# JuliaSmoothOptimizers/LinearOperators.jl

Hardware: AMD Instinct MI355X
Metric: mul! GB/s (frac HBM peak) at n=10^8 fp64; L-BFGS apply/s, 1/2/4/8 GPU (higher is better)
Workload: dtype f64; 1 GPU; opHouseholder(h) 5-arg mul!(res,H,v,1,0), n=100000000 fp64 per GPU (configs[1]); n_per_gpu=100000000, algorithmic_bytes_per_elt=40, devices_visible=1

## Files before the change

### linearoperators.jl_amd/csrc/common.h

```cpp
#pragma once
#include <hip/hip_runtime.h>
#include <atomic>

#include <cstdarg>
#include <cstdint>
#include <cstdio>
#include <cstdlib>
#include <cstring>
#include <initializer_list>
#include <type_traits>
#include <utility>
#include <vector>

#include "../../include/mxlo.h"

#define MXLO_API extern "C" __attribute__((visibility("default")))

namespace mxlo {

constexpr int kBlock = 256;
constexpr int kWave = 64;
constexpr int kMaxRedCols = 128;
constexpr int kQnfMaxCols = 40, kQnfMaxGrid = 256;
constexpr int kQnfSlots = kQnfMaxCols * kQnfMaxGrid;
constexpr int kFusedSlots = 512;
constexpr unsigned long long kSlotEmpty = 0x7FF8DEADBEEF0001ull;
constexpr int kMaxRedBlocks = 4096;
constexpr int kScalarSlots = 8192;

void set_error(const char *fmt, ...);

struct ApiCounters {
  std::atomic<int64_t> n_malloc{0}, n_free{0}, n_h2d{0}, n_d2h{0}, n_d2d{0}, n_d2h_bytes{0}, n_stream_sync{0},
      n_device_sync{0}, n_event_sync{0}, n_memset_async{0}, n_launch{0}, n_blocking_copy{0};
};
inline ApiCounters &api_counters() {
  static ApiCounters c;
  return c;
}
inline void count_copy(size_t bytes, hipMemcpyKind kind, bool blocking) {
  ApiCounters &c = api_counters();
  if (kind == hipMemcpyDeviceToHost) { ++c.n_d2h; c.n_d2h_bytes += (int64_t)bytes; }
  else if (kind == hipMemcpyHostToDevice) ++c.n_h2d;
  else ++c.n_d2d;
  if (blocking) ++c.n_blocking_copy;
}
inline hipError_t counted_memcpy(void *d, const void *s, size_t b, hipMemcpyKind k) {
  count_copy(b, k, true);
  return hipMemcpy(d, s, b, k);
}
inline hipError_t counted_memcpy_async(void *d, const void *s, size_t b, hipMemcpyKind k, hipStream_t st) {
  count_copy(b, k, false);
  return hipMemcpyAsync(d, s, b, k, st);
}
#define hipMalloc(...) (++mxlo::api_counters().n_malloc, hipMalloc(__VA_ARGS__))
#define hipFree(...) (++mxlo::api_counters().n_free, hipFree(__VA_ARGS__))
#define hipHostMalloc(...) (++mxlo::api_counters().n_malloc, hipHostMalloc(__VA_ARGS__))
#define hipHostFree(...) (++mxlo::api_counters().n_free, hipHostFree(__VA_ARGS__))
#define hipMemcpy(...) mxlo::counted_memcpy(__VA_ARGS__)
#define hipMemcpyAsync(...) mxlo::counted_memcpy_async(__VA_ARGS__)
#define hipStreamSynchronize(...) (++mxlo::api_counters().n_stream_sync, hipStreamSynchronize(__VA_ARGS__))
#define hipDeviceSynchronize(...) (++mxlo::api_counters().n_device_sync, hipDeviceSynchronize(__VA_ARGS__))
#define hipEventSynchronize(...) (++mxlo::api_counters().n_event_sync, hipEventSynchronize(__VA_ARGS__))
#define hipMemsetAsync(...) (++mxlo::api_counters().n_memset_async, hipMemsetAsync(__VA_ARGS__))

#define MXLO_HIP(call)                                                                           \
  do {                                                                                           \
    hipError_t e__ = (call);                                                                     \
    if (e__ != hipSuccess) {                                                                     \
      mxlo::set_error("%s failed: %s (%s:%d)", #call, hipGetErrorString(e__), __FILE__, __LINE__); \
      return MXLO_EHIP;                                                                          \
    }                                                                                            \
  } while (0)

#define MXLO_REQUIRE(cond, code, ...)                                                            \
  do {                                                                                           \
    if (!(cond)) {                                                                               \
      mxlo::set_error(__VA_ARGS__);                                                              \
      return (code);                                                                             \
    }                                                                                            \
  } while (0)

#define MXLO_TRY(expr)                                                                           \
  do {                                                                                           \
    int32_t s__ = (expr);                                                                        \
    if (s__ != MXLO_OK) return s__;                                                              \
  } while (0)

inline bool mxlo_trace_on() {
  static const bool on = getenv("MXLO_TRACE") != nullptr;
  return on;
}
#define MXLO_LAUNCH_CHECK()                                                                      \
  do {                                                                                           \
    ++mxlo::api_counters().n_launch;                                                             \
    if (mxlo_trace_on()) {                                                                       \
      fprintf(stderr, "[mxlo] launched %s:%d ... ", __FILE__, __LINE__);                         \
      fflush(stderr);                                                                            \
      (void)hipDeviceSynchronize();                                                              \
      fprintf(stderr, "done\n");                                                                 \
    }                                                                                            \
    hipError_t e__ = hipGetLastError();                                                          \
    if (e__ != hipSuccess) {                                                                     \
      mxlo::set_error("kernel launch failed: %s (%s:%d)", hipGetErrorString(e__), __FILE__,      \
                      __LINE__);                                                                 \
      return MXLO_EHIP;                                                                          \
    }                                                                                            \
  } while (0)
// ... 287 lines not shown
```

### linearoperators.jl_amd/csrc/house_keep.h

```cpp
#pragma once
#include "common.h"
#include "house_keep_plan.h"
#include "stream_kernels.h"

namespace mxlo {

constexpr int kHouseKeepKR = 14;
constexpr int kHouseKeepKL = 4;
constexpr int kHouseKeepUnroll = 4;

template <typename T, typename CA, typename CB, bool BETA0, int KR, int KL>
__global__ void __launch_bounds__(kBlock)
householder_dots_keep_kernel(T *__restrict__ res, const T *__restrict__ h, const T *__restrict__ v, int64_t head,
                             int64_t n, CA alpha, CB beta, HouseKeepPlan pl, unsigned long long *__restrict__ slots,
                             unsigned long long ticks, unsigned *__restrict__ fault, int drop,
                             double *__restrict__ dot_out) {
  constexpr int VEC = Vec16<T>::N, U = kHouseKeepUnroll;
  using V = typename Vec16<T>::type;
  constexpr int64_t CHUNK = (int64_t)kBlock * U;
  extern __shared__ __attribute__((aligned(16))) unsigned char keep_lds[];
  V *lh = reinterpret_cast<V *>(keep_lds), *lx = lh + (int64_t)KL * CHUNK;
  const int tid = threadIdx.x, G = (int)gridDim.x, b = (int)blockIdx.x;
  unsigned long long *epoch = slots + 2 * kFusedSlots;
  const unsigned e = (unsigned)__hip_atomic_load(epoch, __ATOMIC_RELAXED, __HIP_MEMORY_SCOPE_AGENT) & 1u;
  unsigned long long *mine = slots + e * kFusedSlots, *other = slots + (1u - e) * kFusedSlots;
  for (int i = b + tid * G; i < kFusedSlots; i += G * kBlock)
    __hip_atomic_store(other + i, kSlotEmpty, __ATOMIC_RELAXED, __HIP_MEMORY_SCOPE_AGENT);

  const V *hv = reinterpret_cast<const V *>(h + head), *xv = reinterpret_cast<const V *>(v + head);
  V *rv = reinterpret_cast<V *>(res + head);
  double acc = 0.0;
  auto load4 = [&](int64_t round, V (&a)[U], V (&x)[U]) {
    const int64_t base = (round * G + b) * CHUNK + tid;
#pragma unroll
    for (int u = 0; u < U; ++u) {
      x[u] = __builtin_nontemporal_load(xv + base + (int64_t)u * kBlock);
      a[u] = __builtin_nontemporal_load(hv + base + (int64_t)u * kBlock);
    }
  };
  auto fma4 = [&](const V (&a)[U], const V (&x)[U]) {
#pragma unroll
    for (int u = 0; u < U; ++u)
#pragma unroll
      for (int k = 0; k < VEC; ++k) acc = fma((double)a[u][k], (double)x[u][k], acc);
  };
  for (int64_t r = 0; r < pl.first; ++r) {
    V a[U], x[U];
    load4(r, a, x);
    fma4(a, x);
  }
  if constexpr (KL > 0) {
#pragma unroll 1
    for (int q = 0; q < pl.kl; ++q) {
      V a[U], x[U];
      load4(pl.first + q, a, x);
      fma4(a, x);
#pragma unroll
      for (int u = 0; u < U; ++u) {
        lh[(q * U + u) * kBlock + tid] = a[u];
        lx[(q * U + u) * kBlock + tid] = x[u];
      }
    }
  }
  V kh[KR][U], kx[KR][U];
  const int64_t reg0 = pl.first + pl.kl;
#pragma unroll
  for (int q = 0; q < KR; ++q)
    if (q < pl.kr) load4(reg0 + q, kh[q], kx[q]);
#pragma unroll
  for (int q = 0; q < KR; ++q)
    if (q < pl.kr) fma4(kh[q], kx[q]);
  const int64_t rem = pl.rem_vec + (int64_t)b * CHUNK + tid;
#pragma unroll
  for (int u = 0; u < U; ++u) {
    const int64_t i = rem + (int64_t)u * kBlock;
    if (i < pl.nvec) {
      const V x = __builtin_nontemporal_load(xv + i), a = __builtin_nontemporal_load(hv + i);
#pragma unroll
      for (int k = 0; k < VEC; ++k) acc = fma((double)a[k], (double)x[k], acc);
    }
  }
  const int64_t tail0 = head + pl.nvec * VEC, cnt = head + (n - tail0);
  if (b == G - 1 && tid < cnt) {
    const int64_t i = tid < head ? tid : tail0 + (tid - head);
    acc = fma((double)h[i], (double)v[i], acc);
  }

  __shared__ double lds[kBlock / kWave];
  const int wave = tid >> 6, lane = tid & 63;
  acc = wave_sum(acc);
  if (lane == 0) lds[wave] = acc;
  __syncthreads();
  if (tid == 0) {
    const double s = (lds[0] + lds[1]) + (lds[2] + lds[3]);
    unsigned long long bits = (unsigned long long)__double_as_longlong(s);
    if (s != s) bits = kCanonicalNaN;
    if (b != drop) __hip_atomic_store(mine + b, bits, __ATOMIC_RELAXED, __HIP_MEMORY_SCOPE_AGENT);
  }
  double p = 0.0;
  for (int i = tid; i < G; i += kBlock) p += __longlong_as_double((long long)poll_slot(mine + i, ticks, fault, kFaultHouseholder));
  p = wave_sum(p);
  __syncthreads();
  if (lane == 0) lds[wave] = p;
  __syncthreads();
  const double dot = (lds[0] + lds[1]) + (lds[2] + lds[3]);
  if (b == 0 && tid == 0) {
    *dot_out = dot;
    __hip_atomic_store(epoch, (unsigned long long)(1u - e), __ATOMIC_RELAXED, __HIP_MEMORY_SCOPE_AGENT);
  }

  HouseholderOp<T, CA, CB, BETA0> op{alpha, beta, nullptr, T(0)};
  op.c = (T)2 * (T)dot;
  auto update4 = [&](int64_t round, const V (&a)[U], const V (&x)[U]) {
    const int64_t base = (round * G + b) * CHUNK + tid;
    V r[U];
    if constexpr (!BETA0) {
#pragma unroll
      for (int u = 0; u < U; ++u) r[u] = __builtin_nontemporal_load(rv + base + (int64_t)u * kBlock);
    }
#pragma unroll
    for (int u = 0; u < U; ++u) {
      V o;
#pragma unroll
      for (int k = 0; k < VEC; ++k) o[k] = op(a[u][k], x[u][k], BETA0 ? T(0) : r[u][k]);
      __builtin_nontemporal_store(o, rv + base + (int64_t)u * kBlock);
    }
  };
#pragma unroll
  for (int q = 0; q < KR; ++q)
    if (q < pl.kr) update4(reg0 + q, kh[q], kx[q]);
  if constexpr (KL > 0) {
#pragma unroll 1
    for (int q = 0; q < pl.kl; ++q) {
      V a[U], x[U];
#pragma unroll
      for (int u = 0; u < U; ++u) {
        a[u] = lh[(q * U + u) * kBlock + tid];
        x[u] = lx[(q * U + u) * kBlock + tid];
      }
      update4(pl.first + q, a, x);
    }
  }
#pragma unroll
  for (int u = 0; u < U; ++u) {
    const int64_t i = rem + (int64_t)u * kBlock;
    if (i < pl.nvec) {
      const V x = xv[i], a = hv[i];
      V r, o;
      if constexpr (!BETA0) r = rv[i];
#pragma unroll
      for (int k = 0; k < VEC; ++k) o[k] = op(a[k], x[k], BETA0 ? T(0) : r[k]);
      __builtin_nontemporal_store(o, rv + i);
    }
  }
  if (b == G - 1 && tid >= head && tid < cnt) {
    const int64_t i = tail0 + (tid - head);
    res[i] = op(h[i], v[i], BETA0 ? T(0) : res[i]);
  }
}

template <typename T>
static int32_t householder_dots_t(mxlo_ctx *ctx, T *res, const T *h, const T *v, int64_t *n_left, double alpha,
                                  double beta, int32_t flags, double *dot) {
  constexpr int VEC = Vec16<T>::N, KR = kHouseKeepKR, KL = kHouseKeepKL;
  constexpr int64_t CHUNK = (int64_t)kBlock * kHouseKeepUnroll;
  constexpr size_t kLds = (size_t)2 * KL * CHUNK * 16;
  const int64_t n = *n_left;
  const T *cols[1] = {h};
  const int64_t head = common_head<T>({res, h, v});
  bool keep = ctx->tune.house_fused && !ctx->allreduce && ctx->fault_dev && n > ctx->tune.house_inline_n && head >= 0 &&
              n >= 4 * VEC && (int64_t)sizeof(T) * n * 2 >= ctx->tune.nt_min_bytes;
  HouseKeepPlan pl;
  int grid = 0;
  if (keep) {
    const int per_cu = ctx->tune.red_blocks_per_cu > 1 ? 1 : ctx->tune.red_blocks_per_cu;
    grid = grid_for(ctx, (n - head) / VEC, CHUNK, per_cu);
    pl = house_keep_plan(n, head, VEC, grid, CHUNK, KR, KL);
    keep = grid == ctx->num_cu && grid <= kFusedSlots && pl.ok;
  }
  if (!keep) return panel_dots<T>(ctx, cols, 1, v, n, dot);
  bool launched = false;
  MXLO_TRY((dispatch_ab<T>(beta, flags, [&]<typename CA, typename CB, bool B0>() -> int32_t {
    constexpr auto kernel = householder_dots_keep_kernel<T, CA, CB, B0, KR, KL>;
    static std::atomic<int> lds_cap[64];
    const int d = ctx->device & 63;
    int st = kLds > 48 * 1024 ? lds_cap[d].load(std::memory_order_relaxed) : 1;
    if (st == 0) {
      st = hipFuncSetAttribute((const void *)kernel, hipFuncAttributeMaxDynamicSharedMemorySize, (int)kLds) == hipSuccess ? 1 : 2;
      if (st == 2) (void)hipGetLastError();
      lds_cap[d].store(st, std::memory_order_relaxed);
    }
    if (st != 1 || !coresident<kernel>(ctx, grid, kLds)) return MXLO_OK;
    hipLaunchKernelGGL(kernel, dim3(grid), dim3(kBlock), kLds, ctx->stream, res, h, v, head, n, (CA)alpha, (CB)beta, pl,
                       ctx->xslots, fused_timeout_ticks(ctx), ctx->fault_dev, ctx->tune.fused_debug_drop, dot);
    MXLO_LAUNCH_CHECK();
    launched = true;
    return MXLO_OK;
  })));
  if (!launched) return panel_dots<T>(ctx, cols, 1, v, n, dot);
  *n_left = pl.prefix;
  return MXLO_OK;
}

}
```

### linearoperators.jl_amd/csrc/house_keep_plan.h

```cpp
#pragma once
#include <cstdint>

namespace mxlo {

struct HouseKeepPlan {
  bool ok = false;
  int64_t rounds = 0;
  int64_t first = 0;
  int kl = 0, kr = 0;
  int64_t prefix = 0;
  int64_t rem_vec = 0;
  int64_t nvec = 0;
};

inline HouseKeepPlan house_keep_plan(int64_t n, int64_t head, int vec, int64_t grid, int64_t chunk, int KR, int KL) {
  HouseKeepPlan p;
  if (n < head || vec < 1 || grid < 1 || chunk < 1 || KR < 0 || KL < 0) return p;
  p.nvec = (n - head) / vec;
  p.rounds = p.nvec / chunk / grid;
  if (p.rounds < 2) return p;
  const int64_t kept = p.rounds - 1 < (int64_t)KR + KL ? p.rounds - 1 : (int64_t)KR + KL;
  p.kr = (int)(kept < KR ? kept : KR);
  p.kl = (int)(kept - p.kr);
  p.first = p.rounds - kept;
  p.prefix = head + p.first * grid * chunk * vec;
  p.rem_vec = p.rounds * grid * chunk;
  p.ok = kept >= 1;
  return p;
}

}
```

### linearoperators.jl_amd/csrc/leaves.hip

```cpp
#include "common.h"
#include "stream_kernels.h"
#include "house_keep.h"
using namespace mxlo;

#define CHECK_COMMON(name)                                                                       \
  MXLO_REQUIRE(ctx != nullptr, MXLO_EINVAL, name ": ctx is NULL");                               \
  MXLO_REQUIRE(dtype == MXLO_F64 || dtype == MXLO_F32, MXLO_EINVAL, name ": bad dtype %d", dtype)

static inline double eff_beta(int32_t dtype, int32_t flags, double beta) {
  return beta_is_f64(dtype == MXLO_F64 ? 8 : 4, flags) ? beta : (double)(float)beta;
}
static inline double eff_alpha(int32_t dtype, int32_t flags, double alpha) {
  return alpha_is_f64(dtype == MXLO_F64 ? 8 : 4, flags) ? alpha : (double)(float)alpha;
}

template <typename T>
static int32_t fill(mxlo_ctx *ctx, T *p, int64_t n, T c) {
  if (n <= 0) return MXLO_OK;
  if (c == T(0)) {
    MXLO_HIP(hipMemsetAsync(p, 0, sizeof(T) * (size_t)n, ctx->stream));
    return MXLO_OK;
  }
  return launch_map<T, 0, false, false>(ctx, p, (const T *)nullptr, (const T *)nullptr, n,
                                        FillOp<T>{c});
// ... 113 lines not shown
}

namespace {
template <typename T>
__global__ void __launch_bounds__(kBlock)
sum_kernel(const T *__restrict__ v, int64_t n, double *__restrict__ partials) {
  constexpr int VEC = Vec16<T>::N;
  using V = typename Vec16<T>::type;
  double acc = 0.0;
  const int64_t head = (((uintptr_t)v & 15u) == 0) ? 0 : n;
  const int64_t nvec = head == 0 ? n / VEC : 0;
  const V *vv = reinterpret_cast<const V *>(v);
  const int64_t stride = (int64_t)gridDim.x * kBlock;
  int64_t i = (int64_t)blockIdx.x * kBlock + threadIdx.x;
  for (; i + 3 * stride < nvec; i += 4 * stride) {
    const V a = __builtin_nontemporal_load(vv + i), b = __builtin_nontemporal_load(vv + i + stride),
            c = __builtin_nontemporal_load(vv + i + 2 * stride), d = __builtin_nontemporal_load(vv + i + 3 * stride);
#pragma unroll
    for (int e = 0; e < VEC; ++e) acc += ((double)a[e] + (double)b[e]) + ((double)c[e] + (double)d[e]);
  }
  for (; i < nvec; i += stride) {
    const V a = vv[i];
#pragma unroll
    for (int e = 0; e < VEC; ++e) acc += (double)a[e];
  }
  for (int64_t k = nvec * VEC + (int64_t)blockIdx.x * kBlock + threadIdx.x; k < n; k += stride) acc += (double)v[k];
#pragma unroll
  for (int off = 32; off > 0; off >>= 1) acc += __shfl_down(acc, off, 64);
  __shared__ double lds[kBlock / kWave];
  if ((threadIdx.x & 63) == 0) lds[threadIdx.x >> 6] = acc;
  __syncthreads();
  if (threadIdx.x == 0) partials[blockIdx.x] = (lds[0] + lds[1]) + (lds[2] + lds[3]);
}
}

namespace mxlo {
int32_t allreduce_hook(mxlo_ctx *ctx, double *dev, int64_t count);
}

template <typename T>
static int32_t ones_mul_t(mxlo_ctx *ctx, T *res, int64_t nrow, const T *v, int64_t ncol,
                          double alpha, double beta, int32_t flags) {
  double *sum = ctx->scalars;
  if (ncol > 0) {
    const int grid = grid_for(ctx, ncol, kBlock * 8, ctx->tune.red_blocks_per_cu);
    hipLaunchKernelGGL((sum_kernel<T>), dim3(grid), dim3(kBlock), 0, ctx->stream, v, ncol,
                       ctx->partials);
    MXLO_LAUNCH_CHECK();
    MXLO_TRY(finalize_and_reduce(ctx, 1, grid, sum));
  } else {
    MXLO_HIP(hipMemsetAsync(sum, 0, sizeof(double), ctx->stream));
  }
  MXLO_TRY(allreduce_hook(ctx, sum, 1));
  return dispatch_ab<T>(beta, flags, [&]<typename CA, typename CB, bool B0>() -> int32_t {
    OnesOp<T, CA, CB, B0> op{(CA)alpha, (CB)beta, sum, (CA)0};
    return launch_map<T, 0, !B0, false>(ctx, res, (const T *)nullptr, (const T *)nullptr, nrow, op);
  });
}

MXLO_API int32_t mxlo_ones_mul(mxlo_ctx *ctx, int32_t dtype, void *res, int64_t nrow,
                               const void *v, int64_t ncol, double alpha, double beta,
                               int32_t flags) {
  CHECK_COMMON("mxlo_ones_mul");
  MXLO_DEVICE_GUARD(ctx);
  MXLO_REQUIRE(nrow >= 0 && ncol >= 0, MXLO_ESHAPE, "mxlo_ones_mul: negative size");
  alpha = eff_alpha(dtype, flags, alpha);
  beta = eff_beta(dtype, flags, beta);
  if (dtype == MXLO_F64)
    return ones_mul_t<double>(ctx, (double *)res, nrow, (const double *)v, ncol, alpha, beta, flags);
  return ones_mul_t<float>(ctx, (float *)res, nrow, (const float *)v, ncol, alpha, beta, flags);
}

template <typename T>
static int32_t householder_apply_t(mxlo_ctx *ctx, T *res, const T *h, const T *v, int64_t n,
                                   double alpha, double beta, int32_t flags, const double *dot) {
  const bool rev = ctx->tune.house_reverse != 0;
  return dispatch_ab<T>(beta, flags, [&]<typename CA, typename CB, bool B0>() -> int32_t {
    HouseholderOp<T, CA, CB, B0> op{(CA)alpha, (CB)beta, dot, T(0)};
    if (rev) return launch_map<T, 2, !B0, true>(ctx, res, h, v, n, op);
    return launch_map<T, 2, !B0, false>(ctx, res, h, v, n, op);
  });
}

namespace {
template <typename T, typename CA, typename CB, bool BETA0, int VPT, bool ALIGNED>
__global__ void __launch_bounds__(kBlock)
householder_fused_kernel(T *__restrict__ res, const T *__restrict__ h, const T *__restrict__ v, int64_t n, CA alpha,
                         CB beta, unsigned long long *__restrict__ slots, unsigned long long ticks,
                         unsigned *__restrict__ fault, int drop) {
  constexpr int VEC = Vec16<T>::N;
  using V = typename Vec16<T>::type;
  const int tid = threadIdx.x, G = (int)gridDim.x, b = (int)blockIdx.x;
  unsigned long long *epoch = slots + 2 * kFusedSlots;
  const unsigned e = (unsigned)__hip_atomic_load(epoch, __ATOMIC_RELAXED, __HIP_MEMORY_SCOPE_AGENT) & 1u;
  unsigned long long *mine = slots + e * kFusedSlots, *other = slots + (1u - e) * kFusedSlots;
  for (int i = b + tid * G; i < kFusedSlots; i += G * kBlock)
    __hip_atomic_store(other + i, kSlotEmpty, __ATOMIC_RELAXED, __HIP_MEMORY_SCOPE_AGENT);

  T hh[VPT][VEC], vv[VPT][VEC];
  double acc = 0.0;
  const int64_t base = (int64_t)b * kBlock * VPT * VEC;
#pragma unroll
  for (int q = 0; q < VPT; ++q) {
    const int64_t i = base + ((int64_t)q * kBlock + tid) * VEC;
    if (ALIGNED && i + VEC <= n) {
      const V a = *reinterpret_cast<const V *>(h + i), c = *reinterpret_cast<const V *>(v + i);
#pragma unroll
      for (int k = 0; k < VEC; ++k) { hh[q][k] = a[k]; vv[q][k] = c[k]; }
    } else {
#pragma unroll
      for (int k = 0; k < VEC; ++k) {
        hh[q][k] = i + k < n ? h[i + k] : T(0);
        vv[q][k] = i + k < n ? v[i + k] : T(0);
      }
    }
  }
#pragma unroll
  for (int q = 0; q < VPT; ++q)
#pragma unroll
    for (int k = 0; k < VEC; ++k) acc = fma((double)hh[q][k], (double)vv[q][k], acc);

  __shared__ double lds[kBlock / 64];
  const int wave = tid >> 6, lane = tid & 63;
#pragma unroll
  for (int off = 32; off > 0; off >>= 1) acc += __shfl_down(acc, off, 64);
  if (lane == 0) lds[wave] = acc;
  __syncthreads();
  if (tid == 0) {
    const double s = (lds[0] + lds[1]) + (lds[2] + lds[3]);
    unsigned long long bits = (unsigned long long)__double_as_longlong(s);
    if (s != s) bits = kCanonicalNaN;
    if (b != drop) __hip_atomic_store(mine + b, bits, __ATOMIC_RELAXED, __HIP_MEMORY_SCOPE_AGENT);
  }
  double p = 0.0;
  if (tid < G) p = __longlong_as_double((long long)poll_slot(mine + tid, ticks, fault, kFaultHouseholder));
  if (tid + kBlock < G) p += __longlong_as_double((long long)poll_slot(mine + tid + kBlock, ticks, fault, kFaultHouseholder));
#pragma unroll
  for (int off = 32; off > 0; off >>= 1) p += __shfl_down(p, off, 64);
  __syncthreads();
  if (lane == 0) lds[wave] = p;
  __syncthreads();
  const double dot = (lds[0] + lds[1]) + (lds[2] + lds[3]);
  if (b == 0 && tid == 0)
    __hip_atomic_store(epoch, (unsigned long long)(1u - e), __ATOMIC_RELAXED, __HIP_MEMORY_SCOPE_AGENT);

  HouseholderOp<T, CA, CB, BETA0> op{alpha, beta, nullptr, T(0)};
  op.c = (T)2 * (T)dot;
#pragma unroll
  for (int q = 0; q < VPT; ++q) {
    const int64_t i = base + ((int64_t)q * kBlock + tid) * VEC;
    if (ALIGNED && i + VEC <= n) {
      V r;
      if constexpr (!BETA0) r = *reinterpret_cast<const V *>(res + i);
      V o;
#pragma unroll
      for (int k = 0; k < VEC; ++k) o[k] = op(hh[q][k], vv[q][k], BETA0 ? T(0) : r[k]);
      *reinterpret_cast<V *>(res + i) = o;
    } else {
#pragma unroll
      for (int k = 0; k < VEC; ++k)
        if (i + k < n) res[i + k] = op(hh[q][k], vv[q][k], BETA0 ? T(0) : res[i + k]);
    }
  }
}
}

template <typename T>
static inline int64_t fused_grid(int64_t n, int vpt) {
  const int64_t per = (int64_t)kBlock * vpt * Vec16<T>::N;
  return (n + per - 1) / per;
}

template <typename T>
static int32_t householder_fused_t(mxlo_ctx *ctx, T *res, const T *h, const T *v, int64_t n, double alpha, double beta,
                                   int32_t flags, int vpt, bool *launched) {
  const bool aligned = ((((uintptr_t)res) | ((uintptr_t)h) | ((uintptr_t)v)) & 15u) == 0;
  const int grid = (int)fused_grid<T>(n, vpt);
  return dispatch_ab<T>(beta, flags, [&]<typename CA, typename CB, bool B0>() -> int32_t {
    bool fits = true;
    auto go = [&]<int VPT, bool AL>() {
      if (!(fits = coresident<householder_fused_kernel<T, CA, CB, B0, VPT, AL>>(ctx, grid))) return;
      hipLaunchKernelGGL((householder_fused_kernel<T, CA, CB, B0, VPT, AL>), dim3(grid), dim3(kBlock), 0, ctx->stream,
                         res, h, v, n, (CA)alpha, (CB)beta, ctx->xslots, fused_timeout_ticks(ctx), ctx->fault_dev,
                         ctx->tune.fused_debug_drop);
    };
    if (aligned) {
      if (vpt == 2) go.template operator()<2, true>();
      else if (vpt == 4) go.template operator()<4, true>();
      else if (vpt == 8) go.template operator()<8, true>();
      else go.template operator()<16, true>();
    } else {
      if (vpt == 2) go.template operator()<2, false>();
      else if (vpt == 4) go.template operator()<4, false>();
      else if (vpt == 8) go.template operator()<8, false>();
      else go.template operator()<16, false>();
    }
    *launched = fits;
    if (!fits) return MXLO_OK;
    MXLO_LAUNCH_CHECK();
    return MXLO_OK;
  });
}

template <typename T>
static int32_t householder_t(mxlo_ctx *ctx, T *res, const T *h, const T *v, int64_t n,
                             double alpha, double beta, int32_t flags) {
  if (ctx->tune.house_fused && !ctx->allreduce && n > 0 && ctx->fault_dev) {
    MXLO_TRY(fused_fault_check(ctx));
  }
  if (ctx->tune.house_fused && !ctx->allreduce && n > 0 && ctx->fault_dev) {
    const int64_t cap = std::min<int64_t>((int64_t)ctx->num_cu * (ctx->tune.house_fused_per_cu >= 2 ? 2 : 1), kFusedSlots);
    const int64_t cap1 = std::min<int64_t>(ctx->num_cu, kFusedSlots);
    const int vpt = fused_grid<T>(n, 2) <= 16 ? 2 : (fused_grid<T>(n, 4) <= 32 ? 4 : (fused_grid<T>(n, 8) <= cap1 ? 8 : 16));
    if (fused_grid<T>(n, vpt) <= cap) {
      bool launched = false;
      const int32_t st = householder_fused_t<T>(ctx, res, h, v, n, alpha, beta, flags, vpt, &launched);
      if (st != MXLO_OK || launched) return st;
    }
  }
  const T *cols[1] = {h};
  if (!ctx->allreduce && n >= 1 && n <= ctx->tune.house_inline_n) {
    int nb = 0;
    MXLO_TRY(panel_dots_partials<T>(ctx, cols, 1, v, n, &nb));
    const bool rev = ctx->tune.house_reverse != 0;
    return dispatch_ab<T>(beta, flags, [&]<typename CA, typename CB, bool B0>() -> int32_t {
      HouseholderPartialsOp<T, CA, CB, B0> op{(CA)alpha, (CB)beta, ctx->partials, nb, T(0)};
      if (rev) return launch_map<T, 2, !B0, true>(ctx, res, h, v, n, op);
      return launch_map<T, 2, !B0, false>(ctx, res, h, v, n, op);
    });
  }
  double *dot = ctx->scalars;
  MXLO_TRY(householder_dots_t<T>(ctx, res, h, v, &n, alpha, beta, flags, dot));
  return householder_apply_t<T>(ctx, res, h, v, n, alpha, beta, flags, dot);
}

MXLO_API int32_t mxlo_dot(mxlo_ctx *ctx, int32_t dtype, const void *a, const void *b, int64_t n,
                          double *out_dev) {
  CHECK_COMMON("mxlo_dot");
  MXLO_DEVICE_GUARD(ctx);
  MXLO_REQUIRE(n >= 0 && out_dev && (n == 0 || (a && b)), MXLO_EINVAL, "mxlo_dot: bad argument");
  if (dtype == MXLO_F64) {
    const double *cols[1] = {(const double *)a};
    return panel_dots<double>(ctx, cols, 1, (const double *)b, n, out_dev);
  }
  const float *cols[1] = {(const float *)a};
  return panel_dots<float>(ctx, cols, 1, (const float *)b, n, out_dev);
}

MXLO_API int32_t mxlo_householder_apply(mxlo_ctx *ctx, int32_t dtype, void *res, const void *h,
                                        const void *v, int64_t n, double alpha, double beta,
                                        int32_t flags, const double *dot_dev) {
  CHECK_COMMON("mxlo_householder_apply");
  MXLO_DEVICE_GUARD(ctx);
  MXLO_REQUIRE(n >= 0 && dot_dev && (n == 0 || (res && h && v)), MXLO_EINVAL,
               "mxlo_householder_apply: bad argument");
  MXLO_TRY(stage_alias(ctx, res, n * (dtype == MXLO_F64 ? 8 : 4), &v, n * (dtype == MXLO_F64 ? 8 : 4), true,
                       "mxlo_householder_apply"));
  alpha = eff_alpha(dtype, flags, alpha);
  beta = eff_beta(dtype, flags, beta);
  if (dtype == MXLO_F64)
    return householder_apply_t<double>(ctx, (double *)res, (const double *)h, (const double *)v, n,
                                       alpha, beta, flags, dot_dev);
  return householder_apply_t<float>(ctx, (float *)res, (const float *)h, (const float *)v, n, alpha,
                                    beta, flags, dot_dev);
}

MXLO_API int32_t mxlo_householder_mul(mxlo_ctx *ctx, int32_t dtype, void *res, const void *h,
                                      const void *v, int64_t n, double alpha, double beta,
                                      int32_t flags) {
  CHECK_COMMON("mxlo_householder_mul");
  MXLO_DEVICE_GUARD(ctx);
  MXLO_REQUIRE(n >= 0 && (n == 0 || (res && h && v)), MXLO_EINVAL,
               "mxlo_householder_mul: bad argument");
  MXLO_TRY(stage_alias(ctx, res, n * (dtype == MXLO_F64 ? 8 : 4), &v, n * (dtype == MXLO_F64 ? 8 : 4), true,
                       "mxlo_householder_mul"));
  alpha = eff_alpha(dtype, flags, alpha);
  beta = eff_beta(dtype, flags, beta);
  if (dtype == MXLO_F64)
    return householder_t<double>(ctx, (double *)res, (const double *)h, (const double *)v, n, alpha,
                                 beta, flags);
  return householder_t<float>(ctx, (float *)res, (const float *)h, (const float *)v, n, alpha, beta,
                              flags);
}

namespace {
template <typename T>
struct CopyBitsOp {
  __device__ void init() {}
  __device__ T operator()(T x, T, T) const { return x; }
};

typedef unsigned int u32;
typedef unsigned long long u64;
typedef u64 u64x2 __attribute__((ext_vector_type(2)));

template <typename E, bool VECOUT>
__global__ void __launch_bounds__(kBlock)
gather_idx_kernel(E *__restrict__ res, const E *__restrict__ v, const int64_t *__restrict__ idx,
                  int64_t nidx) {
  constexpr int KPT = sizeof(E) >= 16 ? 1 : 16 / (int)sizeof(E);
  constexpr int U = 4;
  typedef long long i64x2 __attribute__((ext_vector_type(2)));
  const int64_t ngroups = (nidx + KPT - 1) / KPT;
  const bool idx_al = (((uintptr_t)idx) & 15u) == 0;
  for (int64_t base = ((int64_t)blockIdx.x * U) * kBlock + threadIdx.x; base < ngroups;
       base += (int64_t)gridDim.x * U * kBlock) {
    int64_t j[U][KPT];
#pragma unroll
    for (int u = 0; u < U; ++u) {
      const int64_t k0 = (base + (int64_t)u * kBlock) * KPT;
      if (KPT >= 2 && idx_al && k0 + KPT <= nidx) {
#pragma unroll
        for (int q = 0; q < KPT; q += 2) {
          const i64x2 t = __builtin_nontemporal_load(reinterpret_cast<const i64x2 *>(idx + k0 + q));
          j[u][q] = t[0] - 1;
          j[u][q + (KPT >= 2 ? 1 : 0)] = t[1] - 1;
// ... 631 lines not shown
```

Baseline: 6989 GB/s.

## Extend keep-in-register Householder kernel to non-temporal-free sizes with virtual-grid accumulators

Generalises the single-pass Householder kernel so a grid pinned to one workgroup per CU can emulate a larger virtual grid. Each block keeps 2 or 4 partial accumulators, selected per round through branchless blends, and publishes one exchange slot per virtual block. Non-temporal loads and stores become a template option, so mid-size inputs below the non-temporal threshold can also use the fused dot-plus-update path instead of a separate dot and apply. The slot array is doubled and the fused-grid cap is decoupled from it. Large inputs keep the previous single-accumulator non-temporal configuration.

```diff
diff --git a/linearoperators.jl_amd/csrc/common.h b/linearoperators.jl_amd/csrc/common.h
--- a/linearoperators.jl_amd/csrc/common.h
+++ b/linearoperators.jl_amd/csrc/common.h
@@ -23,7 +23,7 @@
 constexpr int kMaxRedCols = 128;
 constexpr int kQnfMaxCols = 40, kQnfMaxGrid = 256;
 constexpr int kQnfSlots = kQnfMaxCols * kQnfMaxGrid;
-constexpr int kFusedSlots = 512;
+constexpr int kFusedSlots = 1024;
 constexpr unsigned long long kSlotEmpty = 0x7FF8DEADBEEF0001ull;
 constexpr int kMaxRedBlocks = 4096;
 constexpr int kScalarSlots = 8192;
diff --git a/linearoperators.jl_amd/csrc/house_keep.h b/linearoperators.jl_amd/csrc/house_keep.h
--- a/linearoperators.jl_amd/csrc/house_keep.h
+++ b/linearoperators.jl_amd/csrc/house_keep.h
@@ -9,12 +9,13 @@
 constexpr int kHouseKeepKL = 4;
 constexpr int kHouseKeepUnroll = 4;
 
-template <typename T, typename CA, typename CB, bool BETA0, int KR, int KL>
+template <typename T, typename CA, typename CB, bool BETA0, int KR, int KL, int NV, bool NT>
 __global__ void __launch_bounds__(kBlock)
 householder_dots_keep_kernel(T *__restrict__ res, const T *__restrict__ h, const T *__restrict__ v, int64_t head,
                              int64_t n, CA alpha, CB beta, HouseKeepPlan pl, unsigned long long *__restrict__ slots,
                              unsigned long long ticks, unsigned *__restrict__ fault, int drop,
                              double *__restrict__ dot_out) {
+  static_assert(NV == 1 || NV == 2 || NV == 4, "accumulators per workgroup");
   constexpr int VEC = Vec16<T>::N, U = kHouseKeepUnroll;
   using V = typename Vec16<T>::type;
   constexpr int64_t CHUNK = (int64_t)kBlock * U;
@@ -29,32 +30,91 @@
 
   const V *hv = reinterpret_cast<const V *>(h + head), *xv = reinterpret_cast<const V *>(v + head);
   V *rv = reinterpret_cast<V *>(res + head);
-  double acc = 0.0;
+  auto ld = [](const V *p) -> V {
+    if constexpr (NT) return __builtin_nontemporal_load(p);
+    else return *p;
+  };
+  auto st = [](V o, V *p) {
+    if constexpr (NT) __builtin_nontemporal_store(o, p);
+    else *p = o;
+  };
+  double a0 = 0.0, a1 = 0.0, a2 = 0.0, a3 = 0.0;
+  auto mask = [](int j, int jj) -> unsigned long long {
+    unsigned long long m = j == jj ? ~0ull : 0ull;
+    asm volatile("" : "+v"(m));
+    return m;
+  };
+  auto blend = [](double x, double y, unsigned long long m) -> double {
+    const unsigned long long xb = (unsigned long long)__double_as_longlong(x), yb = (unsigned long long)__double_as_longlong(y);
+    return __longlong_as_double((long long)((yb & m) | (xb & ~m)));
+  };
+  auto pick = [&](int j) -> double {
+    double s = a0;
+    if constexpr (NV >= 2) s = blend(s, a1, mask(j, 1));
+    if constexpr (NV >= 4) {
+      s = blend(s, a2, mask(j, 2));
+      s = blend(s, a3, mask(j, 3));
+    }
+    return s;
+  };
+  auto put = [&](int j, double s) {
+    if constexpr (NV == 1) {
+      a0 = s;
+    } else {
+      a0 = blend(a0, s, mask(j, 0));
+      a1 = blend(a1, s, mask(j, 1));
+      if constexpr (NV >= 4) {
+        a2 = blend(a2, s, mask(j, 2));
+        a3 = blend(a3, s, mask(j, 3));
+      }
+    }
+  };
   auto load4 = [&](int64_t round, V (&a)[U], V (&x)[U]) {
     const int64_t base = (round * G + b) * CHUNK + tid;
 #pragma unroll
     for (int u = 0; u < U; ++u) {
-      x[u] = __builtin_nontemporal_load(xv + base + (int64_t)u * kBlock);
-      a[u] = __builtin_nontemporal_load(hv + base + (int64_t)u * kBlock);
-    }
-  };
-  auto fma4 = [&](const V (&a)[U], const V (&x)[U]) {
+      x[u] = ld(xv + base + (int64_t)u * kBlock);
+      a[u] = ld(hv + base + (int64_t)u * kBlock);
+    }
+  };
+  auto fma4 = [&](const V (&a)[U], const V (&x)[U], double s) -> double {
 #pragma unroll
     for (int u = 0; u < U; ++u)
 #pragma unroll
-      for (int k = 0; k < VEC; ++k) acc = fma((double)a[u][k], (double)x[u][k], acc);
-  };
-  for (int64_t r = 0; r < pl.first; ++r) {
+      for (int k = 0; k < VEC; ++k) s = fma((double)a[u][k], (double)x[u][k], s);
+    return s;
+  };
+  auto fma4_at = [&](int64_t round, const V (&a)[U], const V (&x)[U]) {
+    const int j = house_keep_acc(round, NV);
+    put(j, fma4(a, x, pick(j)));
+  };
+  auto stream = [&](int64_t round, double &s) {
     V a[U], x[U];
-    load4(r, a, x);
-    fma4(a, x);
+    load4(round, a, x);
+    s = fma4(a, x, s);
+  };
+  int64_t r = 0;
+  for (; r + NV <= pl.first; r += NV) {
+    stream(r, a0);
+    if constexpr (NV >= 2) stream(r + 1, a1);
+    if constexpr (NV >= 4) {
+      stream(r + 2, a2);
+      stream(r + 3, a3);
+    }
+  }
+  if constexpr (NV >= 2) {
+    if (r < pl.first) stream(r, a0);
+  }
+  if constexpr (NV >= 4) {
+    if (r + 1 < pl.first) stream(r + 1, a1);
+    if (r + 2 < pl.first) stream(r + 2, a2);
   }
   if constexpr (KL > 0) {
 #pragma unroll 1
     for (int q = 0; q < pl.kl; ++q) {
       V a[U], x[U];
       load4(pl.first + q, a, x);
-      fma4(a, x);
+      fma4_at(pl.first + q, a, x);
 #pragma unroll
       for (int u = 0; u < U; ++u) {
         lh[(q * U + u) * kBlock + tid] = a[u];
@@ -69,41 +129,55 @@
     if (q < pl.kr) load4(reg0 + q, kh[q], kx[q]);
 #pragma unroll
   for (int q = 0; q < KR; ++q)
-    if (q < pl.kr) fma4(kh[q], kx[q]);
+    if (q < pl.kr) fma4_at(reg0 + q, kh[q], kx[q]);
   const int64_t rem = pl.rem_vec + (int64_t)b * CHUNK + tid;
-#pragma unroll
-  for (int u = 0; u < U; ++u) {
-    const int64_t i = rem + (int64_t)u * kBlock;
-    if (i < pl.nvec) {
-      const V x = __builtin_nontemporal_load(xv + i), a = __builtin_nontemporal_load(hv + i);
-#pragma unroll
-      for (int k = 0; k < VEC; ++k) acc = fma((double)a[k], (double)x[k], acc);
-    }
+  {
+    const int jr = house_keep_acc(pl.rounds, NV);
+    double s = pick(jr);
+#pragma unroll
+    for (int u = 0; u < U; ++u) {
+      const int64_t i = rem + (int64_t)u * kBlock;
+      if (i < pl.nvec) {
+        const V x = ld(xv + i), a = ld(hv + i);
+#pragma unroll
+        for (int k = 0; k < VEC; ++k) s = fma((double)a[k], (double)x[k], s);
+      }
+    }
+    put(jr, s);
   }
   const int64_t tail0 = head + pl.nvec * VEC, cnt = head + (n - tail0);
   if (b == G - 1 && tid < cnt) {
     const int64_t i = tid < head ? tid : tail0 + (tid - head);
-    acc = fma((double)h[i], (double)v[i], acc);
-  }
-
-  __shared__ double lds[kBlock / kWave];
+    double &last = NV == 1 ? a0 : (NV == 2 ? a1 : a3);
+    last = fma((double)h[i], (double)v[i], last);
+  }
+
+  __shared__ double lds[NV][kBlock / kWave];
   const int wave = tid >> 6, lane = tid & 63;
-  acc = wave_sum(acc);
-  if (lane == 0) lds[wave] = acc;
+  auto wave_partial = [&](int j, double a) {
+    const double s = wave_sum(a);
+    if (lane == 0) lds[j][wave] = s;
+  };
+  wave_partial(0, a0);
+  if constexpr (NV >= 2) wave_partial(1, a1);
+  if constexpr (NV >= 4) {
+    wave_partial(2, a2);
+    wave_partial(3, a3);
+  }
   __syncthreads();
-  if (tid == 0) {
-    const double s = (lds[0] + lds[1]) + (lds[2] + lds[3]);
+  if (tid < NV) {
+    const double s = (lds[tid][0] + lds[tid][1]) + (lds[tid][2] + lds[tid][3]);
     unsigned long long bits = (unsigned long long)__double_as_longlong(s);
     if (s != s) bits = kCanonicalNaN;
-    if (b != drop) __hip_atomic_store(mine + b, bits, __ATOMIC_RELAXED, __HIP_MEMORY_SCOPE_AGENT);
+    if (b != drop) __hip_atomic_store(mine + house_keep_slot(b, tid, G), bits, __ATOMIC_RELAXED, __HIP_MEMORY_SCOPE_AGENT);
   }
   double p = 0.0;
-  for (int i = tid; i < G; i += kBlock) p += __longlong_as_double((long long)poll_slot(mine + i, ticks, fault, kFaultHouseholder));
+  for (int i = tid; i < NV * G; i += kBlock) p += __longlong_as_double((long long)poll_slot(mine + i, ticks, fault, kFaultHouseholder));
   p = wave_sum(p);
   __syncthreads();
-  if (lane == 0) lds[wave] = p;
+  if (lane == 0) lds[0][wave] = p;
   __syncthreads();
-  const double dot = (lds[0] + lds[1]) + (lds[2] + lds[3]);
+  const double dot = (lds[0][0] + lds[0][1]) + (lds[0][2] + lds[0][3]);
   if (b == 0 && tid == 0) {
     *dot_out = dot;
     __hip_atomic_store(epoch, (unsigned long long)(1u - e), __ATOMIC_RELAXED, __HIP_MEMORY_SCOPE_AGENT);
@@ -113,17 +187,17 @@
   op.c = (T)2 * (T)dot;
   auto update4 = [&](int64_t round, const V (&a)[U], const V (&x)[U]) {
     const int64_t base = (round * G + b) * CHUNK + tid;
-    V r[U];
+    V rr[U];
     if constexpr (!BETA0) {
 #pragma unroll
-      for (int u = 0; u < U; ++u) r[u] = __builtin_nontemporal_load(rv + base + (int64_t)u * kBlock);
+      for (int u = 0; u < U; ++u) rr[u] = ld(rv + base + (int64_t)u * kBlock);
     }
 #pragma unroll
     for (int u = 0; u < U; ++u) {
       V o;
 #pragma unroll
-      for (int k = 0; k < VEC; ++k) o[k] = op(a[u][k], x[u][k], BETA0 ? T(0) : r[u][k]);
-      __builtin_nontemporal_store(o, rv + base + (int64_t)u * kBlock);
+      for (int k = 0; k < VEC; ++k) o[k] = op(a[u][k], x[u][k], BETA0 ? T(0) : rr[u][k]);
+      st(o, rv + base + (int64_t)u * kBlock);
     }
   };
 #pragma unroll
@@ -146,11 +220,11 @@
     const int64_t i = rem + (int64_t)u * kBlock;
     if (i < pl.nvec) {
       const V x = xv[i], a = hv[i];
-      V r, o;
-      if constexpr (!BETA0) r = rv[i];
-#pragma unroll
-      for (int k = 0; k < VEC; ++k) o[k] = op(a[k], x[k], BETA0 ? T(0) : r[k]);
-      __builtin_nontemporal_store(o, rv + i);
+      V rr, o;
+      if constexpr (!BETA0) rr = rv[i];
+#pragma unroll
+      for (int k = 0; k < VEC; ++k) o[k] = op(a[k], x[k], BETA0 ? T(0) : rr[k]);
+      st(o, rv + i);
     }
   }
   if (b == G - 1 && tid >= head && tid < cnt) {
@@ -160,44 +234,49 @@
 }
 
 template <typename T>
-static int32_t householder_dots_t(mxlo_ctx *ctx, T *res, const T *h, const T *v, int64_t *n_left, double alpha,
-                                  double beta, int32_t flags, double *dot) {
+static int32_t householder_keep_t(mxlo_ctx *ctx, T *res, const T *h, const T *v, int64_t *n_left, double alpha,
+                                  double beta, int32_t flags, double *dot, bool above_single, bool *kept) {
   constexpr int VEC = Vec16<T>::N, KR = kHouseKeepKR, KL = kHouseKeepKL;
   constexpr int64_t CHUNK = (int64_t)kBlock * kHouseKeepUnroll;
   constexpr size_t kLds = (size_t)2 * KL * CHUNK * 16;
   const int64_t n = *n_left;
-  const T *cols[1] = {h};
+  *kept = false;
   const int64_t head = common_head<T>({res, h, v});
-  bool keep = ctx->tune.house_fused && !ctx->allreduce && ctx->fault_dev && n > ctx->tune.house_inline_n && head >= 0 &&
-              n >= 4 * VEC && (int64_t)sizeof(T) * n * 2 >= ctx->tune.nt_min_bytes;
-  HouseKeepPlan pl;
-  int grid = 0;
-  if (keep) {
-    const int per_cu = ctx->tune.red_blocks_per_cu > 1 ? 1 : ctx->tune.red_blocks_per_cu;
-    grid = grid_for(ctx, (n - head) / VEC, CHUNK, per_cu);
-    pl = house_keep_plan(n, head, VEC, grid, CHUNK, KR, KL);
-    keep = grid == ctx->num_cu && grid <= kFusedSlots && pl.ok;
-  }
-  if (!keep) return panel_dots<T>(ctx, cols, 1, v, n, dot);
+  if (!(ctx->tune.house_fused && !ctx->allreduce && ctx->fault_dev && head >= 0 && n >= 4 * VEC)) return MXLO_OK;
+  const bool nt = (int64_t)sizeof(T) * n * 2 >= ctx->tune.nt_min_bytes;
+  if (nt ? n <= ctx->tune.house_inline_n : !above_single) return MXLO_OK;
+  const int per_cu = (nt && ctx->tune.red_blocks_per_cu > 1) ? 1 : ctx->tune.red_blocks_per_cu;
+  const int64_t g_virtual = grid_for(ctx, (n - head) / VEC, CHUNK, per_cu);
+  const int grid = ctx->num_cu;
+  const int nv = house_keep_virtual(g_virtual, grid, kFusedSlots);
+  const HouseKeepPlan pl = house_keep_plan(n, head, VEC, grid, CHUNK, KR, KL);
+  if (nv == 0 || (nt && nv != 1) || !pl.ok) return MXLO_OK;
   bool launched = false;
   MXLO_TRY((dispatch_ab<T>(beta, flags, [&]<typename CA, typename CB, bool B0>() -> int32_t {
-    constexpr auto kernel = householder_dots_keep_kernel<T, CA, CB, B0, KR, KL>;
-    static std::atomic<int> lds_cap[64];
-    const int d = ctx->device & 63;
-    int st = kLds > 48 * 1024 ? lds_cap[d].load(std::memory_order_relaxed) : 1;
-    if (st == 0) {
-      st = hipFuncSetAttribute((const void *)kernel, hipFuncAttributeMaxDynamicSharedMemorySize, (int)kLds) == hipSuccess ? 1 : 2;
-      if (st == 2) (void)hipGetLastError();
-      lds_cap[d].store(st, std::memory_order_relaxed);
-    }
-    if (st != 1 || !coresident<kernel>(ctx, grid, kLds)) return MXLO_OK;
-    hipLaunchKernelGGL(kernel, dim3(grid), dim3(kBlock), kLds, ctx->stream, res, h, v, head, n, (CA)alpha, (CB)beta, pl,
-                       ctx->xslots, fused_timeout_ticks(ctx), ctx->fault_dev, ctx->tune.fused_debug_drop, dot);
-    MXLO_LAUNCH_CHECK();
-    launched = true;
-    return MXLO_OK;
+    auto go = [&]<int NV, bool NT>() -> int32_t {
+      constexpr auto kernel = householder_dots_keep_kernel<T, CA, CB, B0, KR, KL, NV, NT>;
+      static std::atomic<int> lds_cap[64];
+      const int d = ctx->device & 63;
+      int st = kLds > 48 * 1024 ? lds_cap[d].load(std::memory_order_relaxed) : 1;
+      if (st == 0) {
+        st = hipFuncSetAttribute((const void *)kernel, hipFuncAttributeMaxDynamicSharedMemorySize, (int)kLds) == hipSuccess ? 1 : 2;
+        if (st == 2) (void)hipGetLastError();
+        lds_cap[d].store(st, std::memory_order_relaxed);
+      }
+      if (st != 1 || !coresident<kernel>(ctx, grid, kLds)) return MXLO_OK;
+      hipLaunchKernelGGL(kernel, dim3(grid), dim3(kBlock), kLds, ctx->stream, res, h, v, head, n, (CA)alpha, (CB)beta, pl,
+                         ctx->xslots, fused_timeout_ticks(ctx), ctx->fault_dev, ctx->tune.fused_debug_drop, dot);
+      MXLO_LAUNCH_CHECK();
+      launched = true;
+      return MXLO_OK;
+    };
+    if (nt) return go.template operator()<1, true>();
+    if (nv == 1) return go.template operator()<1, false>();
+    if (nv == 2) return go.template operator()<2, false>();
+    return go.template operator()<4, false>();
   })));
-  if (!launched) return panel_dots<T>(ctx, cols, 1, v, n, dot);
+  if (!launched) return MXLO_OK;
+  *kept = true;
   *n_left = pl.prefix;
   return MXLO_OK;
 }
diff --git a/linearoperators.jl_amd/csrc/house_keep_plan.h b/linearoperators.jl_amd/csrc/house_keep_plan.h
--- a/linearoperators.jl_amd/csrc/house_keep_plan.h
+++ b/linearoperators.jl_amd/csrc/house_keep_plan.h
@@ -29,4 +29,15 @@
   return p;
 }
 
+
+constexpr int house_keep_virtual(int64_t g_virtual, int64_t grid, int64_t slots) {
+  if (grid < 1 || g_virtual < grid || g_virtual > slots || g_virtual % grid) return 0;
+  const int64_t v = g_virtual / grid;
+  return v == 1 || v == 2 || v == 4 ? (int)v : 0;
 }
+
+constexpr int house_keep_acc(int64_t round, int nv) { return (int)(round & (int64_t)(nv - 1)); }
+
+constexpr int64_t house_keep_slot(int64_t b, int j, int64_t grid) { return b + (int64_t)j * grid; }
+
+}
diff --git a/linearoperators.jl_amd/csrc/leaves.hip b/linearoperators.jl_amd/csrc/leaves.hip
--- a/linearoperators.jl_amd/csrc/leaves.hip
+++ b/linearoperators.jl_amd/csrc/leaves.hip
@@ -219,6 +219,8 @@
   });
 }
 
+constexpr int kFusedMaxGrid = 2 * kBlock;
+static_assert(kFusedMaxGrid <= kFusedSlots, "one exchange slot per workgroup");
 namespace {
 template <typename T, typename CA, typename CB, bool BETA0, int VPT, bool ALIGNED>
 __global__ void __launch_bounds__(kBlock)
@@ -345,16 +347,24 @@
   if (ctx->tune.house_fused && !ctx->allreduce && n > 0 && ctx->fault_dev) {
     MXLO_TRY(fused_fault_check(ctx));
   }
+  bool above_single = false;
   if (ctx->tune.house_fused && !ctx->allreduce && n > 0 && ctx->fault_dev) {
-    const int64_t cap = std::min<int64_t>((int64_t)ctx->num_cu * (ctx->tune.house_fused_per_cu >= 2 ? 2 : 1), kFusedSlots);
-    const int64_t cap1 = std::min<int64_t>(ctx->num_cu, kFusedSlots);
+    const int64_t cap = std::min<int64_t>((int64_t)ctx->num_cu * (ctx->tune.house_fused_per_cu >= 2 ? 2 : 1), kFusedMaxGrid);
+    const int64_t cap1 = std::min<int64_t>(ctx->num_cu, kFusedMaxGrid);
     const int vpt = fused_grid<T>(n, 2) <= 16 ? 2 : (fused_grid<T>(n, 4) <= 32 ? 4 : (fused_grid<T>(n, 8) <= cap1 ? 8 : 16));
     if (fused_grid<T>(n, vpt) <= cap) {
       bool launched = false;
       const int32_t st = householder_fused_t<T>(ctx, res, h, v, n, alpha, beta, flags, vpt, &launched);
       if (st != MXLO_OK || launched) return st;
-    }
-  }
+    } else {
+      above_single = true;
+    }
+  }
+  double *dot = ctx->scalars;
+  bool kept = false;
+  int64_t n_left = n;
+  MXLO_TRY(householder_keep_t<T>(ctx, res, h, v, &n_left, alpha, beta, flags, dot, above_single, &kept));
+  if (kept) return householder_apply_t<T>(ctx, res, h, v, n_left, alpha, beta, flags, dot);
   const T *cols[1] = {h};
   if (!ctx->allreduce && n >= 1 && n <= ctx->tune.house_inline_n) {
     int nb = 0;
@@ -366,8 +376,7 @@
       return launch_map<T, 2, !B0, false>(ctx, res, h, v, n, op);
     });
   }
-  double *dot = ctx->scalars;
-  MXLO_TRY(householder_dots_t<T>(ctx, res, h, v, &n, alpha, beta, flags, dot));
+  MXLO_TRY(panel_dots<T>(ctx, cols, 1, v, n, dot));
   return householder_apply_t<T>(ctx, res, h, v, n, alpha, beta, flags, dot);
 }
 
```

Result: no change. 6986 GB/s (-0.0%).

## Keep a cache-sized fraction of h resident between dot and update passes

Applied to the files above, without the earlier changes.

In the kept-form dot kernel, a diagonal subset of chunks (fraction q/16, sized to the cache budget derived from nt_min_bytes) loads h with normal cached loads instead of nontemporal ones, so those lines can stay in the last-level cache. A new update kernel uses the same chunk-to-diagonal mapping to reread those h chunks through the cache and streams the rest. The aim is to cut HBM reads of h in the second pass. The cost is a branch per chunk, an added dependence on cache retention between launches, and a new update path with a stricter chunk-alignment requirement.

```diff
diff --git a/linearoperators.jl_amd/csrc/house_keep.h b/linearoperators.jl_amd/csrc/house_keep.h
--- a/linearoperators.jl_amd/csrc/house_keep.h
+++ b/linearoperators.jl_amd/csrc/house_keep.h
@@ -8,13 +8,22 @@
 constexpr int kHouseKeepKR = 14;
 constexpr int kHouseKeepKL = 4;
 constexpr int kHouseKeepUnroll = 4;
+static_assert(kHouseKeepUnroll == kStreamUnroll, "the dot launch and the update launch count the same chunks");
+
+constexpr int kHouseResidentNum = 14;
+static_assert(kHouseResidentNum >= 0 && kHouseResidentNum <= 16);
+#define MXLO_POLICY_SIDE(tag) asm volatile("; h loads: " tag ::: "memory")
+struct HouseResident {
+  int q = 0;
+  int grid = 0;
+};
 
 template <typename T, typename CA, typename CB, bool BETA0, int KR, int KL>
 __global__ void __launch_bounds__(kBlock)
 householder_dots_keep_kernel(T *__restrict__ res, const T *__restrict__ h, const T *__restrict__ v, int64_t head,
                              int64_t n, CA alpha, CB beta, HouseKeepPlan pl, unsigned long long *__restrict__ slots,
                              unsigned long long ticks, unsigned *__restrict__ fault, int drop,
-                             double *__restrict__ dot_out) {
+                             double *__restrict__ dot_out, int rq) {
   constexpr int VEC = Vec16<T>::N, U = kHouseKeepUnroll;
   using V = typename Vec16<T>::type;
   constexpr int64_t CHUNK = (int64_t)kBlock * U;
@@ -32,10 +41,22 @@
   double acc = 0.0;
   auto load4 = [&](int64_t round, V (&a)[U], V (&x)[U]) {
     const int64_t base = (round * G + b) * CHUNK + tid;
-#pragma unroll
-    for (int u = 0; u < U; ++u) {
-      x[u] = __builtin_nontemporal_load(xv + base + (int64_t)u * kBlock);
-      a[u] = __builtin_nontemporal_load(hv + base + (int64_t)u * kBlock);
+    if (house_resident_diag((int)((round + b) & 15), rq)) {
+      MXLO_POLICY_SIDE("resident");
+#pragma unroll
+      for (int u = 0; u < U; ++u) {
+        x[u] = __builtin_nontemporal_load(xv + base + (int64_t)u * kBlock);
+        a[u] = hv[base + (int64_t)u * kBlock];
+      }
+      MXLO_POLICY_SIDE("resident, issued");
+    } else {
+      MXLO_POLICY_SIDE("streamed");
+#pragma unroll
+      for (int u = 0; u < U; ++u) {
+        x[u] = __builtin_nontemporal_load(xv + base + (int64_t)u * kBlock);
+        a[u] = __builtin_nontemporal_load(hv + base + (int64_t)u * kBlock);
+      }
+      MXLO_POLICY_SIDE("streamed, issued");
     }
   };
   auto fma4 = [&](const V (&a)[U], const V (&x)[U]) {
@@ -161,7 +182,7 @@
 
 template <typename T>
 static int32_t householder_dots_t(mxlo_ctx *ctx, T *res, const T *h, const T *v, int64_t *n_left, double alpha,
-                                  double beta, int32_t flags, double *dot) {
+                                  double beta, int32_t flags, double *dot, HouseResident *rs) {
   constexpr int VEC = Vec16<T>::N, KR = kHouseKeepKR, KL = kHouseKeepKL;
   constexpr int64_t CHUNK = (int64_t)kBlock * kHouseKeepUnroll;
   constexpr size_t kLds = (size_t)2 * KL * CHUNK * 16;
@@ -179,6 +200,7 @@
     keep = grid == ctx->num_cu && grid <= kFusedSlots && pl.ok;
   }
   if (!keep) return panel_dots<T>(ctx, cols, 1, v, n, dot);
+  const int rq = house_resident_q((int64_t)sizeof(T) * n, ctx->tune.nt_min_bytes / 16 * kHouseResidentNum);
   bool launched = false;
   MXLO_TRY((dispatch_ab<T>(beta, flags, [&]<typename CA, typename CB, bool B0>() -> int32_t {
     constexpr auto kernel = householder_dots_keep_kernel<T, CA, CB, B0, KR, KL>;
@@ -192,14 +214,86 @@
     }
     if (st != 1 || !coresident<kernel>(ctx, grid, kLds)) return MXLO_OK;
     hipLaunchKernelGGL(kernel, dim3(grid), dim3(kBlock), kLds, ctx->stream, res, h, v, head, n, (CA)alpha, (CB)beta, pl,
-                       ctx->xslots, fused_timeout_ticks(ctx), ctx->fault_dev, ctx->tune.fused_debug_drop, dot);
+                       ctx->xslots, fused_timeout_ticks(ctx), ctx->fault_dev, ctx->tune.fused_debug_drop, dot, rq);
     MXLO_LAUNCH_CHECK();
     launched = true;
     return MXLO_OK;
   })));
   if (!launched) return panel_dots<T>(ctx, cols, 1, v, n, dot);
   *n_left = pl.prefix;
+  *rs = HouseResident{rq, grid};
   return MXLO_OK;
 }
 
-}
+template <typename T, typename CA, typename CB, bool BETA0, bool REVERSE, bool NT>
+__global__ void __launch_bounds__(kBlock)
+householder_update_resident_kernel(T *__restrict__ res, const T *__restrict__ h, const T *__restrict__ v, int64_t head,
+                                   int64_t nchunks, int64_t dots_grid, int rq, HouseholderOp<T, CA, CB, BETA0> op) {
+  constexpr int VEC = Vec16<T>::N, U = kStreamUnroll;
+  using V = typename Vec16<T>::type;
+  constexpr int64_t CHUNK = (int64_t)kBlock * U;
+  op.init();
+  const int tid = threadIdx.x;
+  V *rv = reinterpret_cast<V *>(res + head);
+  const V *hv = reinterpret_cast<const V *>(h + head), *xv = reinterpret_cast<const V *>(v + head);
+  for (int64_t ch = blockIdx.x; ch < nchunks; ch += gridDim.x) {
+    const int64_t c = REVERSE ? (nchunks - 1 - ch) : ch;
+    const int64_t base = c * CHUNK + tid;
+    V a[U], x[U], r[U];
+    if (house_resident_chunk(c, dots_grid, rq)) {
+      MXLO_POLICY_SIDE("resident");
+#pragma unroll
+      for (int u = 0; u < U; ++u) {
+        a[u] = hv[base + (int64_t)u * kBlock];
+        x[u] = ldg<NT>(xv + base + (int64_t)u * kBlock);
+        if constexpr (!BETA0) r[u] = ldg<NT>(rv + base + (int64_t)u * kBlock);
+      }
+      MXLO_POLICY_SIDE("resident, issued");
+    } else {
+      MXLO_POLICY_SIDE("streamed");
+#pragma unroll
+      for (int u = 0; u < U; ++u) {
+        a[u] = ldg<NT>(hv + base + (int64_t)u * kBlock);
+        x[u] = ldg<NT>(xv + base + (int64_t)u * kBlock);
+        if constexpr (!BETA0) r[u] = ldg<NT>(rv + base + (int64_t)u * kBlock);
+      }
+      MXLO_POLICY_SIDE("streamed, issued");
+    }
+#pragma unroll
+    for (int u = 0; u < U; ++u) {
+      V o;
+#pragma unroll
+      for (int k = 0; k < VEC; ++k) o[k] = op(a[u][k], x[u][k], BETA0 ? T(0) : r[u][k]);
+      stg<NT>(rv + base + (int64_t)u * kBlock, o);
+    }
+  }
+  if (blockIdx.x == gridDim.x - 1 && tid < head) res[tid] = op(h[tid], v[tid], BETA0 ? T(0) : res[tid]);
+}
+
+template <typename T>
+static int32_t householder_apply_resident_t(mxlo_ctx *ctx, T *res, const T *h, const T *v, int64_t n, double alpha,
+                                            double beta, int32_t flags, const double *dot, HouseResident rs) {
+  constexpr int VEC = Vec16<T>::N;
+  constexpr int64_t CHUNK = (int64_t)kBlock * kStreamUnroll;
+  const int64_t head = common_head<T>({res, h, v}), nchunks = (n - head) / VEC / CHUNK;
+  MXLO_REQUIRE(head >= 0 && rs.grid > 0 && head + nchunks * CHUNK * VEC == n, MXLO_ESTATE,
+               "householder: the prefix of the kept form is not the scalar head and whole chunks");
+  const bool rev = ctx->tune.house_reverse != 0;
+  int64_t g = nchunks;
+  if (ctx->tune.blocks_per_cu > 0 && g > (int64_t)ctx->num_cu * ctx->tune.blocks_per_cu) g = (int64_t)ctx->num_cu * ctx->tune.blocks_per_cu;
+  const int grid = (int)(g > 0x7fffffffLL ? 0x7fffffffLL : (g < 1 ? 1 : g));
+  return dispatch_ab<T>(beta, flags, [&]<typename CA, typename CB, bool B0>() -> int32_t {
+    HouseholderOp<T, CA, CB, B0> op{(CA)alpha, (CB)beta, dot, T(0)};
+    const bool nt = (int64_t)sizeof(T) * n * (B0 ? 3 : 4) >= ctx->tune.nt_min_bytes;
+    auto go = [&]<bool REV, bool NT>() {
+      hipLaunchKernelGGL((householder_update_resident_kernel<T, CA, CB, B0, REV, NT>), dim3(grid), dim3(kBlock), 0,
+                         ctx->stream, res, h, v, head, nchunks, (int64_t)rs.grid, rs.q, op);
+    };
+    if (rev) nt ? go.template operator()<true, true>() : go.template operator()<true, false>();
+    else nt ? go.template operator()<false, true>() : go.template operator()<false, false>();
+    MXLO_LAUNCH_CHECK();
+    return MXLO_OK;
+  });
+}
+
+}
diff --git a/linearoperators.jl_amd/csrc/house_keep_plan.h b/linearoperators.jl_amd/csrc/house_keep_plan.h
--- a/linearoperators.jl_amd/csrc/house_keep_plan.h
+++ b/linearoperators.jl_amd/csrc/house_keep_plan.h
@@ -29,4 +29,16 @@
   return p;
 }
 
+
+constexpr int house_resident_q(int64_t h_bytes, int64_t cache_bytes) {
+  if (cache_bytes <= 0 || h_bytes < 0) return 0;
+  if (h_bytes <= cache_bytes) return 16;
+  return (int)(cache_bytes / ((h_bytes + 15) / 16));
 }
+
+constexpr bool house_resident_diag(int t, int q) { return (t * q) % 16 >= 16 - q; }
+constexpr bool house_resident_chunk(int64_t c, int64_t grid, int q) {
+  return house_resident_diag((int)(((c / grid) + (c % grid)) % 16), q);
+}
+
+}
diff --git a/linearoperators.jl_amd/csrc/leaves.hip b/linearoperators.jl_amd/csrc/leaves.hip
--- a/linearoperators.jl_amd/csrc/leaves.hip
+++ b/linearoperators.jl_amd/csrc/leaves.hip
@@ -367,8 +367,8 @@
     });
   }
   double *dot = ctx->scalars;
-  MXLO_TRY(householder_dots_t<T>(ctx, res, h, v, &n, alpha, beta, flags, dot));
-  return householder_apply_t<T>(ctx, res, h, v, n, alpha, beta, flags, dot);
+  HouseResident rs; MXLO_TRY(householder_dots_t<T>(ctx, res, h, v, &n, alpha, beta, flags, dot, &rs));
+  return rs.q > 0 ? householder_apply_resident_t<T>(ctx, res, h, v, n, alpha, beta, flags, dot, rs) : householder_apply_t<T>(ctx, res, h, v, n, alpha, beta, flags, dot);
 }
 
 MXLO_API int32_t mxlo_dot(mxlo_ctx *ctx, int32_t dtype, const void *a, const void *b, int64_t n,
```

Measured after the change: 6849 GB/s before, 7272 GB/s after (median of 6 runs). 1.06x the previous value.
